# gsgen3d/gsgen

Measured on AMD Instinct MI355X. Metric: fwd+bwd renders/sec (800x800, 100k Gaussians), higher is better.
Workload: dtype f32

## Files before the change

gsgen_amd/_capi.py:

```python
import ctypes as C
import os

_HERE = os.path.dirname(os.path.abspath(__file__))
DEFAULT_LIB = os.environ.get("GSGEN_HIP_LIB") or os.path.join(_HERE, "lib", "libgsgen_hip.so")

u32, f32, vp, i32, sz = C.c_uint32, C.c_float, C.c_void_p, C.c_int, C.c_size_t



class ShView(C.Structure):
    _fields_ = [("mean", vp), ("cov", vp), ("start", vp), ("end", vp), ("gaussian_ids", vp),
                ("tile_order", vp), ("topleft", vp), ("c2w", vp), ("bg_rgb", vp),
                ("pixel_size_x", f32), ("pixel_size_y", f32), ("out", vp), ("T", vp),
                ("segment_workspace", vp), ("grad_out", vp), ("grad_mean", vp), ("grad_cov", vp), ("route_report", vp),
                ("no_fallback", u32), ("pixel_size_dev", vp)]


class RgbdView(C.Structure):
    _fields_ = [("mean", vp), ("cov", vp), ("depth", vp), ("start", vp), ("end", vp), ("gaussian_ids", vp),
                ("tile_order", vp), ("topleft", vp), ("pixel_size_x", f32), ("pixel_size_y", f32), ("out6", vp),
                ("T", vp), ("grad_out6", vp), ("grad_mean", vp), ("grad_cov", vp), ("grad_chan6", vp),
                ("grad_rgb", vp), ("grad_depth", vp), ("grad_opacity", vp), ("grad_depth2", vp),
                ("out_rgb", vp), ("out_depth", vp), ("out_opacity", vp), ("out_depth2", vp), ("bg_rgb", vp), ("grad_bg", vp),
                ("depth_variance", u32), ("chol", vp), ("pixel_size_dev", vp)]


class GeometryView(C.Structure):
    _fields_ = [("cam", vp), ("mean2d", vp), ("cov2d", vp), ("depth", vp), ("mask", vp), ("gaussian_ids", vp),
                ("start", vp), ("end", vp), ("total", vp), ("workspace", vp), ("workspace_bytes", sz), ("D_cap", u32),
                ("zero_grad_mean2d", vp), ("zero_grad_cov2d", vp), ("zero_grad_chan6", vp), ("pair_report", vp), ("chol", vp),
# ... 113 lines not shown
    "gsgen_image_loss_backward": [vp, vp, u32, u32, u32, u32, u32, f32, i32, vp, vp, vp, sz, vp],
    "gsgen_marching_cubes": [vp, u32, u32, u32, f32, vp, u32, vp, u32, vp, vp, sz, vp],
    "gsgen_depth_loss_forward": [vp, vp, sz, vp, sz, u32, u32, vp, vp, sz, vp],
    "gsgen_depth_loss_backward": [vp, vp, sz, vp, sz, u32, u32, vp, vp, vp, vp, sz, vp],
}
OPTIONAL_SIZE_FUNCS = {
    "gsgen_knn_workspace_bytes": [u32, u32],
    "gsgen_knn_query_workspace_bytes": [u32, u32, u32],
    "gsgen_density_grid_workspace_bytes": [u32, u32],
    "gsgen_fps_workspace_bytes": [u32, u32, u32, u32, i32],
    "gsgen_image_loss_workspace_bytes": [u32, u32, u32, u32, u32, i32],
    "gsgen_marching_cubes_workspace_bytes": [u32, u32, u32],
    "gsgen_depth_loss_workspace_bytes": [u32, u32],
}
EXPORTS = sorted(list(SIGNATURES) + list(SIZE_FUNCS) + list(PTR_FUNCS) + list(OPTIONAL_SIGNATURES) + list(OPTIONAL_SIZE_FUNCS)
                 + ["gsgen_version", "gsgen_error_string", "gsgen_kernel_variant", "gsgen_sh_poly_applies", "gsgen_emit_stage_capacity"])


class GsgenError(RuntimeError):
    pass


class Lib:
    def __init__(self, path=None):
        path = path or DEFAULT_LIB
        if not os.path.exists(path):
            raise ImportError(
                f"{path} not found: build the HIP extension first (python -m gsgen_amd.build). "
                "gsgen_amd has no CPU fallback.")
        self.path = path
        if path == DEFAULT_LIB or "libgsgen_hip" in os.path.basename(path):
# ... 35 lines not shown
        def call(*args):
            rc = fn(*args)
            if rc != 0:
                raise GsgenError(f"{name} failed: {err(rc).decode()} (code {rc})")
        call.__name__ = name
        return call

    def version(self):
        return self.cdll.gsgen_version().decode()

    def emit_stage_capacity(self):
        fn = self.cdll.gsgen_emit_stage_capacity
        fn.restype, fn.argtypes = u32, []
        return int(fn())

    def sh_poly_applies(self, sh_l1_bound, max_pixel_size, bands=4):
        fn = self.cdll.gsgen_sh_poly_applies
        fn.argtypes, fn.restype = [f32, f32, u32], i32
        return bool(fn(float(sh_l1_bound), float(max_pixel_size), int(bands)))

    def kernel_variant(self, stage, bands=4, n_segments=1):
        fn = self.cdll.gsgen_kernel_variant
        fn.argtypes, fn.restype = [C.c_char_p, u32, u32, C.c_char_p, sz], i32
        buf = C.create_string_buffer(192)
        n = fn(stage.encode(), bands, n_segments, buf, len(buf))
        if n <= 0:
            raise ValueError(f"unknown compositing stage {stage!r}")
        return buf.value.decode()


# ... 11 lines not shown
```

gsgen_amd/batch.py:

```python
import ctypes

import numpy as np
import torch

from . import _capi
from . import renderer as R
from .renderer import _p, PairListOverflow


ACTIVATION_CODES = {"nothing": 0, "exp": 1, "sigmoid": 2, "abs": 3, "relu": 4, "softplus": 5, "biased_relu": 6, "biased_abs": 7}
TORCH_ACTIVATIONS = {"nothing": lambda x: x, "exp": torch.exp, "sigmoid": torch.sigmoid, "abs": torch.abs, "relu": torch.relu,
                     "softplus": torch.nn.functional.softplus, "biased_relu": lambda x: torch.relu(x) + 1e-3,
                     "biased_abs": lambda x: torch.abs(x) + 1e-3}

_EXT = [False]


def _batch_ext():
    if _EXT[0] is False:
        import glob
        import importlib.util
        import os
        hits = glob.glob(os.path.join(os.path.dirname(os.path.abspath(__file__)), "ext", "_gsbatch.*.so"))
        mod = None
# ... 47 lines not shown
        out_p, T_p = out.data_ptr(), T.data_ptr()
        kind = "sh" if C > 0 else "rgb"
        gsh = torch.empty(br._Np + (col.numel() + 3) // 4 * 4, device=dev, dtype=torch.float32)
        with _on(dev):
            parts = br._fork(B)
            views = br._geometry(kind, B, parts, mean, qvec, svec, gsh, stats)
            bg_p = _p(bg_rgb)
            cis = br._cis
            if C > 0:
                rr, nf = br._route_args
                for i in range(B):
                    ci, v = cis[i], views[i]
                    v.pixel_size_x, v.pixel_size_y = 1.0 / ci.fx, 1.0 / ci.fy
                    v.T, v.bg_rgb, v.out = T_p + 4 * H * W * i, bg_p, out_p + 12 * H * W * i
                    v.route_report, v.no_fallback = rr, nf
            else:
                for i in range(B):
                    ci, v = cis[i], views[i]
                    v.pixel_size_x, v.pixel_size_y = 1.0 / ci.fx, 1.0 / ci.fy
                    v.T, v.out6 = T_p + 4 * H * W * i, out_p + 12 * H * W * i
            nth, ntw = br.slots[0].nth, br.slots[0].ntw
            for k, (lo, n, s) in enumerate(parts):
                if C > 0:
                    lib.vol_render_sh_batch_routed(n, _sub(views, lo, n), N, _p(col), _p(alpha), 16, nth, ntw, H, W, C,
                                                   thresh, br.segments, _p(br._sh_bound), _p(br._sh_rows), _p(br._bws[k]), s)
                else:
                    lib.vol_render_rgb_batch(n, _sub(views, lo, n), N, _p(col), _p(alpha), 16, nth, ntw, H, W, thresh,
                                             _p(br._bws[k]), s)
            br._join(parts)
        if C == 0 and bg_rgb is not None:
# ... 162 lines not shown
class BatchRenderer:

    def __init__(self, N, W, H, device, max_batch, D_cap=None, segments=1, strict=False, pipeline=False, device_cameras=False):
        self.N, self.W, self.H, self.device = N, W, H, torch.device(device)
        self.device_cameras = bool(device_cameras)
        self.segments = int(segments)
        self.strict = bool(strict)
        if pipeline not in ("auto", True, False):
            raise ValueError("pipeline: 'auto', True or False")
        self.pipeline = pipeline
        self._totals = torch.zeros(max_batch, device=device, dtype=torch.int32)
        self._report = R.PairCountReport(max_batch)
        self._route = R.PairCountReport(1)
        self._route_clean = 0
        self._route_args = (None, 0)
        self.strict = self.strict or self._report.unmapped
        self._gen = np.zeros(1, np.int64)
        self._plans = {}
        self.use_ext = True
        self._sh_bound = self._sh_rows = None
        self._table_cache = {}
        self._depths = torch.empty(max_batch, N, device=device, dtype=torch.float32)
        self.slots = [R.FrameBuffers(N, W, H, device, D_cap=D_cap, segments=self.segments, total=self._totals[i:i + 1],
                                     depth=self._depths[i].view(N, 1), report=(self._report, i), strict=self.strict)
                      for i in range(max_batch)]
        self._ptr_tabs = {}
        self._side = None
        self._ev = None
        lib = _capi.load()
        self._Np = (N + 3) // 4 * 4
# ... 305 lines not shown
        self._sh_bound = self._sh_rows = None
        if int(C) == 4 and sh_basis == "auto":
            if sh_l1_bound is not None:
                if not (isinstance(sh_l1_bound, torch.Tensor) and sh_l1_bound.is_cuda and sh_l1_bound.dtype == torch.float32
                        and sh_l1_bound.numel() == 1):
                    raise ValueError("sh_l1_bound: a 1-float CUDA tensor (the bound lives on the device; "
                                     "renderer.sh_l1_bound_device computes it)")
                if verify_bound:
                    R.verify_sh_l1_bound(col, sh_l1_bound)
                self._sh_bound = sh_l1_bound
            else:
                self._sh_rows = self._measure_bound(col)
                self._sh_bound = self._smax if self._sh_rows is self._rows else None
        self._begin_batch(B)
        self._route_args = self._route_mode() if (int(C) == 4 and self._sh_rows is not None) else (None, 0)
        fast = self._plan("sh" if int(C) > 0 else "rgb", B)
        if fast is not None:
            self._last_parts = [(0, B)]
            va = fast[1]
            va["pixel_size_x"][:B] = 1.0 / self._intr[:B, 0]
            va["pixel_size_y"][:B] = 1.0 / self._intr[:B, 1]
            if int(C) > 0:
                va["route_report"][:B] = self._route_args[0] or 0
                va["no_fallback"][:B] = self._route_args[1]
            out, T = _batch_ext().render(fast[0], mean, qvec, svec, alpha, col, bg_rgb, int(C), float(thresh), bool(detach_depth),
                                         self._sh_bound, self._sh_rows, *self._stats_args(stats))
            return out, T
        return _render_batch.apply(mean, qvec, svec, alpha, col, cams, self, B, int(C), bg_rgb, float(thresh),
                                   bool(detach_depth), stats)

    def _route_mode(self):
        rep = self._route
        if rep.ptr(0) is None:
            return None, 0
        seen = int(rep._np[0, 0])
        rep._np[0, 0] = 0
        self._route_clean = 0 if seen else self._route_clean + 1
        return rep.ptr(0), 1 if (self._route_clean >= 3 and not self.device_cameras) else 0

# ... 54 lines not shown
```

gsgen_amd/csrc/composite.hip:

```cpp
#include "composite_common.hpp"
#include <stdio.h>
#include <string.h>
#include <string>
#include <type_traits>
#include <vector>

namespace gs {

template <int MODE, int CB, int KB = kBatch, bool WITH_COL = true>
struct Stage {
  using TR = Traits<MODE, CB>;
  float mx[KB], my[KB], a[KB];
  float c0[KB], c1[KB], c2[KB], c3[KB];
  float p0[KB], p1[KB], p2[KB];
  int id[KB];
  alignas(16) float col[WITH_COL ? KB * TR::NCOLP : 4];
};

template <int MODE, int CB, int NT, int KB = kBatch, bool SCALE = false, bool WITH_COL = true>
__device__ __forceinline__ void stage_batch(Stage<MODE, CB, KB, WITH_COL> &S, const CompParams &p, int list_base,
                                            int nb) {
  using TR = Traits<MODE, CB>;
  const int t = (int)threadIdx.x;
  static_assert(KB <= NT, "one thread per staged record");
// ... 419 lines not shown
  }
}
template <int NT>
__device__ __forceinline__ uint32_t exact_tier_mask(const CompParams &p, const int *ids, int nb, int t, uint32_t *slot) {
  bool bad = false;
  if (p.sh_rows != nullptr && t < nb) bad = !poly_row_ok(p.sh_rows[ids[t]], fmaxf(fabsf(p.psx), fabsf(p.psy)));
  const uint32_t m = (uint32_t)__ballot((int)bad);
  if constexpr (NT == 64) {
    (void)slot;
    return m;
  } else {
    if (t == 0) *slot = m;
    return 0u;
  }
}
template <int CB, bool POLY>
struct FwdShVecShared {
  static constexpr int KB = POLY ? 32 : kBatch;
  Stage<MODE_SH, CB, KB, !POLY> S;
  alignas(16) float Vs[POLY ? kPolyNB * 16 : 4];
  alignas(16) float Ws[POLY ? KB * 3 * kPolyStride : 4];
  uint32_t exact_mask;
  float tay_ok[POLY ? KB * 3 : 1];
};
template <int CB, int PPL, int NB, bool PERSIST = false, bool TRACK = true>
__device__ __forceinline__ void composite_fwd_sh_vec_tile(const CompParams &p, uint32_t bid, FwdShVecShared<CB, (NB > 0)> &sm) {
  static_assert(PPL == 4 || PPL == 2, "pixel pairs: 2 or 4 pixels per lane");
  constexpr bool POLY = NB > 0;
  static_assert(!POLY || (NB == kPolyNB && CB == 4), "polynomial basis: SH degree 3");
  constexpr int MODE = MODE_SH;
  using TR = Traits<MODE, CB>;
  constexpr int NT = 256 / PPL, ROWS = NT / 16, NP = PPL / 2;
  constexpr int CCP = POLY ? NB : TR::CCP, NPAIR = CCP / 2;
  constexpr int KB = FwdShVecShared<CB, POLY>::KB;
  auto &S = sm.S;
  float *const Vs = sm.Vs;
  float *const Ws = sm.Ws;
  int tx, ty;
  if (!block_tile(p, tx, ty, bid)) return;
  const int tile = ty * p.ntw + tx;
  const int st = p.start[tile];
  const int n = (st < 0) ? 0 : (p.end[tile] - st);
  const int t = tile_thread_index<PERSIST>();
  const int lx = t & 15, ly0 = t >> 4;
  const int gx = tx * kTile + lx;

  bool valid[PPL];
  int gy[PPL], stop[PPL];
#pragma unroll
  for (int j = 0; j < PPL; ++j) {
    gy[j] = ty * kTile + ly0 + j * ROWS;
    valid[j] = (gx < p.W) && (gy[j] < p.H);
    stop[j] = valid[j] ? n : 0;
  }
  if constexpr (POLY) {
    if (t == 0 && p.tile_flags != nullptr) p.tile_flags[tile] = 0;
  }
  const bool has_bg = p.bg != nullptr;
  float bgv[3] = {0.0f, 0.0f, 0.0f};
  if (has_bg) { bgv[0] = p.bg[0]; bgv[1] = p.bg[1]; bgv[2] = p.bg[2]; }
  if (st == kListOverflow) {
#pragma unroll
    for (int j = 0; j < PPL; ++j)
      if (valid[j]) poison_pixel<3>(p, (size_t)gy[j] * p.W + gx);
    return;
  }
  if (n == 0) {
    if (p.bg != nullptr || p.fill_empty) {
#pragma unroll
      for (int j = 0; j < PPL; ++j)
        if (valid[j]) {
// ... 12 lines not shown
  }

  const float px = pixel_coord(p.topleft[0], gx, p.psx);
  v2f py2[NP];
#pragma unroll
  for (int j = 0; j < PPL; ++j) py2[j >> 1][j & 1] = pixel_coord(p.topleft[1], gy[j], p.psy);
  v2f Yp[POLY ? 1 : PPL][POLY ? 1 : NPAIR];
  const float pu = poly_offset(lx);
  const v2f pu2 = splat2(pu);
  v2f pv2[NP];
#pragma unroll
  for (int jp = 0; jp < NP; ++jp) pv2[jp] = v2f{poly_offset(ly0 + (2 * jp) * ROWS), poly_offset(ly0 + (2 * jp + 1) * ROWS)};
  if constexpr (POLY) {
    static_assert(KB * 3 * kPolyNB >= kPolyNodes * 16, "node scratch fits the coefficient buffer");
    poly_tile_setup<NT>(p, tx, ty, Ws, Vs);
  } else {
    float R[9];
#pragma unroll
    for (int i = 0; i < 9; ++i) R[i] = p.rot[i];
#pragma unroll
    for (int j = 0; j < PPL; ++j) {
      const float pyj = py2[j >> 1][j & 1];
      float Yf[CCP];
      sh_basis_of_pixel<CB>(R, px, pyj, Yf);
#pragma unroll
      for (int k = 0; k < NPAIR; ++k) Yp[j][k] = v2f{Yf[2 * k], Yf[2 * k + 1]};
      __builtin_amdgcn_sched_barrier(0);
    }
  }

  v2f acc2[NP][3], Tr2[NP];
#pragma unroll
  for (int jp = 0; jp < NP; ++jp) {
#pragma unroll
    for (int c = 0; c < 3; ++c) acc2[jp][c] = v2f{0.0f, 0.0f};
    Tr2[jp] = v2f{valid[2 * jp] ? 1.0f : -1.0f, valid[2 * jp + 1] ? 1.0f : -1.0f};
  }
  auto alive = [&](int j) { return !(Tr2[j >> 1][j & 1] < p.thresh); };
  const bool seg_out = p.nseg > 1 && p.ckpt != nullptr;
  const bool track_stop = TRACK && p.stop != nullptr;

  uint32_t exact_mask = 0u;
  uint32_t tay_mask = 0u;
  for (int base = 0; base < n; base += KB) {
    const int nb = min(KB, n - base);
    if (base > 0) __syncthreads();
    stage_batch<MODE, CB, NT, KB, true, !POLY>(S, p, st + base, nb);
    if constexpr (POLY) {
      if (p.sh_rows != nullptr) {
        exact_mask = exact_tier_mask<NT>(p, S.id, nb, t, &sm.exact_mask);
        __syncthreads();
        if constexpr (NT != 64) exact_mask = sm.exact_mask;
        exact_mask = (uint32_t)__builtin_amdgcn_readfirstlane((int)exact_mask);
        if (__popcll((unsigned long long)exact_mask) * kExactTierShare > nb) {
          if (t == 0 && p.route_report != nullptr) report_crowded_tile(p.route_report);
          if (!p.no_fallback) {
            if (t == 0 && p.tile_flags != nullptr) p.tile_flags[tile] = 1;
            return;
          }
        }
      } else {
        exact_mask = 0u;
        __syncthreads();
      }
      poly_transform<NT, KB>(p.col, S.id, Vs, Ws, nb, sm.tay_ok);
      __syncthreads();
      tay_mask = (uint32_t)__builtin_amdgcn_readfirstlane((int)(taylor_mask(sm.tay_ok, nb) & ~exact_mask));
      taylor_convert<NT>(Ws, tay_mask, nb);
      __syncthreads();
    } else {
      __syncthreads();
    }

    for (int g = 0; g < nb; ++g) {
      bool any_alive = false;
#pragma unroll
      for (int j = 0; j < PPL; ++j) any_alive |= alive(j);
      if (!wave_any(any_alive)) break;
      const int e_idx = base + g;
      if (seg_out && (e_idx % kSegLen) == 0 && e_idx > 0 && e_idx / kSegLen < p.nseg) {
#pragma unroll
        for (int j = 0; j < PPL; ++j)
          p.ckpt[((size_t)tile * p.nseg + e_idx / kSegLen) * 256 + (ly0 + j * ROWS) * 16 + lx] =
              make_float4(Tr2[j >> 1][j & 1], acc2[j >> 1][0][j & 1], acc2[j >> 1][1][j & 1], acc2[j >> 1][2][j & 1]);
// ... 102 lines not shown
          const bool was[2] = {alive(2 * jp), alive(2 * jp + 1)};
          Tr2[jp] = Tr2[jp] * one_minus2(ag2[jp]);
#pragma unroll
          for (int e = 0; e < 2; ++e)
            if (was[e] && !alive(2 * jp + e)) stop[2 * jp + e] = base + g + 1;
        }
      } else {
#pragma unroll
        for (int jp = 0; jp < NP; ++jp) Tr2[jp] = Tr2[jp] * one_minus2(ag2[jp]);
      }
    }
    bool any_alive = false;
#pragma unroll
    for (int j = 0; j < PPL; ++j) any_alive |= alive(j);
    if (__syncthreads_or((int)any_alive) == 0) break;
  }

#pragma unroll
  for (int j = 0; j < PPL; ++j) {
    if (!valid[j]) continue;
    const size_t pix = (size_t)gy[j] * p.W + gx;
    const float Tj = Tr2[j >> 1][j & 1];
    float *o = p.out + 3 * pix;
#pragma unroll
    for (int c = 0; c < 3; ++c) {
      const float a = acc2[j >> 1][c][j & 1];
      o[c] = has_bg ? a + bgv[c] * Tj : a;
    }
    if (p.T != nullptr) p.T[pix] = Tj;
  }
// ... 98 lines not shown
      const CompParams *pp = &plist[view];
      const PixelSizes<PSD> ps = view_pixel_sizes<PSD>(*pp);
      if (per_tile ? !tile_flagged(*pp, b - base) : poly_route(pp->sh_bound, ps.x(), ps.y())) continue;
      const CompParams p = view_params<PSD>(*pp, ps);
      composite_fwd_sh_vec_tile<4, PPL, 0, true>(p, b - base, sm);
      __syncthreads();
    }
  } else if constexpr (NB == kPolyNB && BATCH) {
    __shared__ FwdShVecShared<4, true> sm;
    const CompParams *pp = &plist[batch_view(p_arg, bid)];
    const PixelSizes<PSD> ps = view_pixel_sizes<PSD>(*pp);
    const bool view_ok = pp->sh_bound != nullptr && poly_route(pp->sh_bound, ps.x(), ps.y());
    if (pp->sh_rows == nullptr && !view_ok) return;
    CompParams p = view_params<PSD>(*pp, ps);
    if (view_ok) p.sh_rows = nullptr;
    composite_fwd_sh_vec_tile<4, PPL, kPolyNB, false, TRACK>(p, bid, sm);
  } else {
    const CompParams *pp = BATCH ? &plist[batch_view(p_arg, bid)] : &p_arg;
    const CompParams p = view_params<PSD>(*pp, view_pixel_sizes<PSD>(*pp));
    __shared__ FwdShVecShared<CB, (NB > 0)> sm;
    composite_fwd_sh_vec_tile<CB, PPL, NB>(p, bid, sm);
  }
}

template <int MODE, int CB, int PPL, int TS>
__global__ void __launch_bounds__(TS * TS / PPL)
k_composite_bwd_pixel(CompParams p) {
  const uint32_t bid = blockIdx.x, grid = gridDim.x;
  using TR = Traits<MODE, CB>;
  constexpr int NT = TS * TS / PPL;
  static_assert(NT >= kBatch && NT % 64 == 0, "a staging round needs one thread per record");
// ... 210 lines not shown
    if (__syncthreads_or((int)any_alive) == 0) break;
  }
}


template <int CB, int PPL, bool POLY>
struct BwdShVecShared {
  static constexpr int KB = 32;
  static constexpr int NT = 256 / PPL, NP = PPL / 2;
  Stage<MODE_SH, CB, KB, !POLY> S;
  v2f go_s[!POLY ? 3 * NP * NT : 1];
  alignas(16) float Vs[POLY ? kPolyNB * 16 : 4];
  alignas(16) float Ws[POLY ? KB * 3 * kPolyStride : 4];
  float gw_s[POLY ? 3 * 8 : 1];
  float tay_ok[POLY ? KB * 3 : 1];
};
template <int CB, int PPL, int NB, bool PERSIST = false, bool MOM = false>
__device__ __forceinline__ void composite_bwd_sh_vec_tile(const CompParams &p, uint32_t bid, uint32_t grid,
                                                          BwdShVecShared<CB, PPL, (NB > 0)> &sm) {
  static_assert(PPL == 4 || PPL == 2, "pixel pairs: 2 or 4 pixels per lane");
  constexpr bool POLY = NB > 0;
  static_assert(!POLY || (NB == kPolyNB && CB == 4 && PPL == 4), "polynomial basis: SH degree 3, one wavefront per tile");
  constexpr int MODE = MODE_SH;
  using TR = Traits<MODE, CB>;
  constexpr int NT = 256 / PPL, ROWS = NT / 16, NP = PPL / 2;
  constexpr int CCP = POLY ? NB : TR::CCP, NPAIR = CCP / 2, NSH = 3 * CCP;
  static_assert(NSH % 2 == 0, "component layout");
  constexpr int KB = BwdShVecShared<CB, PPL, POLY>::KB;
  auto &S = sm.S;
  v2f *const go_s = sm.go_s;
  float *const Vs = sm.Vs;
  float *const Ws = sm.Ws;
  float *const gw_s = sm.gw_s;
  const int nseg = p.nseg > 1 ? p.nseg : 1;
  const uint32_t tiles_grid = grid / (uint32_t)nseg;
  const int seg = (int)(bid / tiles_grid);
// ... 35 lines not shown
  if constexpr (TR::CCP != TR::CC) {
    for (int e = t; e < KB * TR::NCOLP; e += NT) S.col[e] = 0.0f;
    __syncthreads();
  }

  v2f Yp[POLY ? 1 : PPL][POLY ? 1 : NPAIR];
  float *geo_base = nullptr;
  uint32_t geo_stride = 0u;
  const float pu = poly_offset(lx);
  const v2f pu2 = splat2(pu);
  v2f pv2[NP];
#pragma unroll
  for (int jp = 0; jp < NP; ++jp) pv2[jp] = v2f{poly_offset(ly0 + (2 * jp) * ROWS), poly_offset(ly0 + (2 * jp + 1) * ROWS)};
  if constexpr (POLY) {
    static_assert(!POLY || KB * 3 * kPolyNB >= kPolyNodes * 16, "node scratch fits the coefficient buffer");
    poly_tile_setup<NT>(p, tx, ty, Ws, Vs);
    {
      const int comp = sep16_comp(lane), cls = comp >> 3, slot = comp & 7;
      if (sep16_owner(lane)) {
        if (cls < 3 && slot == 6) {
          geo_base = cls == 0 ? p.g_mean : p.g_cov + (cls == 1 ? 0 : (MOM ? 2 : 3));
          geo_stride = cls == 0 ? 2u : 4u;
        } else if (cls == 3) {
          geo_base = slot == 0 ? p.g_mean + 1 : (slot == 1 ? p.g_cov + 1 : p.g_alpha);
          geo_stride = slot == 0 ? 2u : (slot == 1 ? 4u : 1u);
        }
      } else if (!MOM && cls == 3 && slot == 1) {
        geo_base = p.g_cov + 2;
        geo_stride = 4u;
      }
    }
// ... 32 lines not shown
    R2[jp] = fma2(go2[jp][2], rem2[jp][2], fma2(go2[jp][1], rem2[jp][1], go2[jp][0] * rem2[jp][0]));
    pvsq2[jp] = pv2[jp] * pv2[jp];
  }
  if constexpr (!POLY) {
#pragma unroll
    for (int jp = 0; jp < NP; ++jp)
#pragma unroll
      for (int c = 0; c < 3; ++c) go_s[(c * NP + jp) * NT + t] = go2[jp][c];
  }
  auto alive = [&](int j) { return !(Tr2[j >> 1][j & 1] < p.thresh); };

  uint32_t exact_mask = 0u, tay_mask = 0u;
  for (int base = e_lo; base < e_hi; base += KB) {
    const int nb = min(KB, e_hi - base);
    if (base > e_lo) __syncthreads();
    stage_batch<MODE, CB, NT, KB, true, !POLY>(S, p, st + base, nb);
    __syncthreads();
    if constexpr (POLY) {
      exact_mask = (uint32_t)__builtin_amdgcn_readfirstlane((int)exact_tier_mask<NT>(p, S.id, nb, t, nullptr));
      poly_transform<NT, KB>(p.col, S.id, Vs, Ws, nb, sm.tay_ok);
      __syncthreads();
      tay_mask = (uint32_t)__builtin_amdgcn_readfirstlane((int)(taylor_mask(sm.tay_ok, nb) & ~exact_mask));
      taylor_convert<NT>(Ws, tay_mask, nb);
      __syncthreads();
    }

    for (int g = 0; g < nb; ++g) {
      bool any_alive = false;
#pragma unroll
      for (int j = 0; j < PPL; ++j) any_alive |= alive(j);
      if (!wave_any(any_alive)) break;

      auto uni = [&](float v) { return !POLY ? wave_uniform(v) : v; };
      const float r_mx = uni(S.mx[g]), r_my = uni(S.my[g]), r_a = uni(S.a[g]), r_c0 = uni(S.c0[g]), r_c1 = uni(S.c1[g]),
                  r_c2 = uni(S.c2[g]), r_c3 = uni(S.c3[g]), r_p0 = uni(S.p0[g]), r_p1 = uni(S.p1[g]);
      const float x = px - r_mx;
      v2f y2[NP], G2[NP], ag2[NP], tx2[NP], ty2[NP];
      bool any_con = false;
      float guard_dist = 0.0f;
// ... 270 lines not shown
      const CompParams *pp = &plist[view];
      const PixelSizes<PSD> ps = view_pixel_sizes<PSD>(*pp);
      if (per_tile ? !tile_flagged(*pp, (b - base) % tiles_grid) : poly_route(pp->sh_bound, ps.x(), ps.y())) continue;
      const CompParams p = view_params<PSD>(*pp, ps);
      composite_bwd_sh_vec_tile<4, 4, 0, true, MOM>(p, b - base, per, sm);
      __syncthreads();
    }
  } else if constexpr (NB == kPolyNB && BATCH) {
    __shared__ BwdShVecShared<4, 4, true> sm;
    const CompParams *pp = &plist[batch_view(p_arg, bid, &grid)];
    const PixelSizes<PSD> ps = view_pixel_sizes<PSD>(*pp);
    const bool view_ok = pp->sh_bound != nullptr && poly_route(pp->sh_bound, ps.x(), ps.y());
    if (pp->sh_rows == nullptr && !view_ok) return;
    CompParams p = view_params<PSD>(*pp, ps);
    if (view_ok) p.sh_rows = nullptr;
    composite_bwd_sh_vec_tile<4, 4, kPolyNB, false, MOM>(p, bid, grid, sm);
  } else {
    const CompParams *pp = BATCH ? &plist[batch_view(p_arg, bid, &grid)] : &p_arg;
    const CompParams p = view_params<PSD>(*pp, view_pixel_sizes<PSD>(*pp));
    __shared__ BwdShVecShared<CB, PPL, (NB > 0)> sm;
    composite_bwd_sh_vec_tile<CB, PPL, NB, false, MOM>(p, bid, grid, sm);
  }
}

template <int MODE, bool BATCH = false>
__global__ void __launch_bounds__(64) GS_WAVES_PER_EU(6)
k_composite_fwd_chan_vec(CompParams p_arg, ViewPack<BATCH> pack) {
  const CompParams *plist = pack.table();
  static_assert(MODE == MODE_RGB || MODE == MODE_SCALAR || MODE == MODE_RGBD, "post-activation channel modes");
  uint32_t bid = blockIdx.x;
  const CompParams p = BATCH ? view_params(plist[batch_view(p_arg, bid)]) : p_arg;
// ... 750 lines not shown
    p.stop = reinterpret_cast<int *>(p.ckpt + (size_t)n_tiles_h * n_tiles_w * 256 * n_segments);
  }
  hipStream_t s = (hipStream_t)stream;
  switch (C) {
    case 1: return launch_fwd<MODE_SH, 1>(p, s);
    case 2: return launch_fwd<MODE_SH, 2>(p, s);
    case 3: return launch_fwd<MODE_SH, 3>(p, s);
    default: return launch_fwd<MODE_SH, 4>(p, s);
  }
}

static int fill_view_params(uint32_t n_views, const gsgen_sh_view *views, const float *sh_coeffs,
                            const float *alpha, float *g_sh, float *g_alpha, uint32_t ntw, uint32_t nth,
                            uint32_t H, uint32_t W, float thresh, uint32_t n_segments, bool backward,
                            const float *sh_bound, std::vector<CompParams> &ps, const float *sh_rows = nullptr,
                            uint8_t *tile_flags = nullptr) {
  ps.assign(n_views, CompParams{});
  for (uint32_t b = 0; b < n_views; ++b) {
    const gsgen_sh_view &v = views[b];
    if (!v.start || !v.end || !v.out || !v.c2w) return GSGEN_EINVAL;
    if ((v.tile_order == nullptr) != (views[0].tile_order == nullptr)) return GSGEN_EINVAL;
    if (n_segments > 1 && v.segment_workspace == nullptr) return GSGEN_EINVAL;
    if (backward && (!v.grad_out || !v.grad_mean || !v.grad_cov)) return GSGEN_EINVAL;
    if ((v.pixel_size_dev == nullptr) != (views[0].pixel_size_dev == nullptr)) return GSGEN_EINVAL;
    CompParams &p = ps[b];
    p.mean = v.mean; p.cov = v.cov; p.col = sh_coeffs; p.alpha = alpha;
    p.start = v.start; p.end = v.end; p.ids = v.gaussian_ids; p.topleft = v.topleft; p.rot = v.c2w;
    p.ntw = (int)ntw; p.nth = (int)nth; p.H = (int)H; p.W = (int)W;
    p.psx = v.pixel_size_x; p.psy = v.pixel_size_y; p.thresh = thresh;
    p.ps_dev = v.pixel_size_dev;
    p.tile_order = v.tile_order;
    p.n_hi = 0x7fffffff;
    p.sh_bound = sh_bound;
    p.sh_rows = sh_rows;
    p.tile_flags = (sh_rows != nullptr && tile_flags != nullptr) ? tile_flags + (size_t)b * ntw * nth : nullptr;
    p.route_report = sh_rows != nullptr ? v.route_report : nullptr;
    p.no_fallback = (sh_rows != nullptr && views[0].no_fallback) ? 1 : 0;
    if (backward) {
      p.final_img = v.out; p.grad_out = v.grad_out;
      p.g_mean = v.grad_mean; p.g_cov = v.grad_cov; p.g_col = g_sh; p.g_alpha = g_alpha;
    } else {
      p.bg = v.bg_rgb; p.out = v.out; p.T = v.T;
      p.fill_empty = 1;
    }
    if (n_segments > 1) {
      p.nseg = (int)n_segments;
      p.ckpt = reinterpret_cast<float4 *>(v.segment_workspace);
      p.stop = reinterpret_cast<int *>(p.ckpt + (size_t)nth * ntw * 256 * n_segments);
    }
  }
  return 0;
}
// ... 163 lines not shown
  return sh_l1_pass<true>(N, sh_coeffs, C, nullptr, bound, n_violations, (hipStream_t)stream);
}

int gsgen_sh_poly_applies(float sh_l1_bound, float max_pixel_size, uint32_t C) {
  return (C == 4 && poly_ok(sh_l1_bound, max_pixel_size)) ? 1 : 0;
}

static bool batch_can_be_polynomial(const std::vector<CompParams> &ps) {
  if (!ps.empty() && ps[0].ps_dev != nullptr) return true;
  for (const CompParams &p : ps)
    if (poly_ok(1.0f / 16.0f, fmaxf(fabsf(p.psx), fabsf(p.psy)))) return true;
  return false;
}

size_t gsgen_sh_batch_workspace_bytes(uint32_t n_views) { return 2 * (size_t)n_views * sizeof(CompParams); }
size_t gsgen_sh_batch_workspace_bytes_routed(uint32_t n_views, uint32_t n_tiles) {
  return gsgen_sh_batch_workspace_bytes(n_views) + (((size_t)n_views * n_tiles + 15u) & ~(size_t)15u);
}

int gsgen_vol_render_sh_batch(uint32_t n_views, const gsgen_sh_view *views, uint32_t N,
                              const float *sh_coeffs, const float *alpha, uint32_t tile_size,
                              uint32_t n_tiles_h, uint32_t n_tiles_w, uint32_t H, uint32_t W, uint32_t C,
                              float thresh, uint32_t n_segments, void *batch_workspace,
                              gsgen_stream_t stream) {
  return gsgen_vol_render_sh_batch_bounded(n_views, views, N, sh_coeffs, alpha, tile_size, n_tiles_h, n_tiles_w, H, W, C,
                                           thresh, n_segments, nullptr, batch_workspace, stream);
}

int gsgen_vol_render_sh_batch_bounded(uint32_t n_views, const gsgen_sh_view *views, uint32_t N,
                                      const float *sh_coeffs, const float *alpha, uint32_t tile_size,
                                      uint32_t n_tiles_h, uint32_t n_tiles_w, uint32_t H, uint32_t W, uint32_t C,
                                      float thresh, uint32_t n_segments, const float *sh_l1_bound, void *batch_workspace,
// ... 3 lines not shown
}

int gsgen_vol_render_sh_batch_routed(uint32_t n_views, const gsgen_sh_view *views, uint32_t N,
                                     const float *sh_coeffs, const float *alpha, uint32_t tile_size,
                                     uint32_t n_tiles_h, uint32_t n_tiles_w, uint32_t H, uint32_t W, uint32_t C,
                                     float thresh, uint32_t n_segments, const float *sh_l1_bound, const float *sh_row_bounds,
                                     void *batch_workspace, gsgen_stream_t stream) {
  if (tile_size != 16) return GSGEN_EUNSUPPORTED;
  if (C < 1 || C > 4) return GSGEN_EUNSUPPORTED;
  if (n_views == 0) return 0;
  if (!views || !batch_workspace) return GSGEN_EINVAL;
  if (n_views > 65535) return GSGEN_EINVAL;
  (void)N;
  std::vector<CompParams> ps;
  uint8_t *flags = reinterpret_cast<uint8_t *>(batch_workspace) + gsgen_sh_batch_workspace_bytes(n_views);
  if (int e = fill_view_params(n_views, views, sh_coeffs, alpha, nullptr, nullptr, n_tiles_w, n_tiles_h, H, W,
                               thresh, n_segments, false, C == 4 ? sh_l1_bound : nullptr, ps, C == 4 ? sh_row_bounds : nullptr, flags))
    return e;
  const bool bounded = C == 4 && (sh_l1_bound != nullptr || sh_row_bounds != nullptr) && batch_can_be_polynomial(ps);
  if (!bounded)
    for (CompParams &p : ps) { p.sh_bound = nullptr; p.sh_rows = nullptr; p.tile_flags = nullptr; }
  hipStream_t s = (hipStream_t)stream;
  return launch_fwd_sh_batch((int)C, ps.data(), n_views, s, bounded);
}

int gsgen_vol_render_backward_sh_batch(uint32_t n_views, const gsgen_sh_view *views, uint32_t N,
                                       const float *sh_coeffs, const float *alpha, float *grad_sh_coeffs,
                                       float *grad_alpha, uint32_t tile_size, uint32_t n_tiles_h,
                                       uint32_t n_tiles_w, uint32_t H, uint32_t W, uint32_t C, float thresh,
                                       uint32_t n_segments, void *batch_workspace, gsgen_stream_t stream) {
  return gsgen_vol_render_backward_sh_batch_bounded(n_views, views, N, sh_coeffs, alpha, grad_sh_coeffs, grad_alpha, tile_size,
                                                    n_tiles_h, n_tiles_w, H, W, C, thresh, n_segments, nullptr, batch_workspace,
                                                    stream);
}

int gsgen_vol_render_backward_sh_batch_bounded(uint32_t n_views, const gsgen_sh_view *views, uint32_t N,
// ... 8 lines not shown
}

static int backward_sh_batch_routed(bool moments, uint32_t n_views, const gsgen_sh_view *views, uint32_t N,
                                    const float *sh_coeffs, const float *alpha, float *grad_sh_coeffs,
                                    float *grad_alpha, uint32_t tile_size, uint32_t n_tiles_h,
                                    uint32_t n_tiles_w, uint32_t H, uint32_t W, uint32_t C, float thresh,
                                    uint32_t n_segments, const float *sh_l1_bound, const float *sh_row_bounds,
                                    void *batch_workspace, gsgen_stream_t stream) {
  if (tile_size != 16) return GSGEN_EUNSUPPORTED;
  if (C < 1 || C > 4) return GSGEN_EUNSUPPORTED;
  if (n_views == 0 || N == 0) return 0;
  if (!views || !batch_workspace || !grad_sh_coeffs || !grad_alpha) return GSGEN_EINVAL;
  if (n_views > 65535) return GSGEN_EINVAL;
  std::vector<CompParams> ps;
  uint8_t *flags = reinterpret_cast<uint8_t *>(batch_workspace) + gsgen_sh_batch_workspace_bytes(n_views);
  if (int e = fill_view_params(n_views, views, sh_coeffs, alpha, grad_sh_coeffs, grad_alpha, n_tiles_w,
                               n_tiles_h, H, W, thresh, n_segments, true, C == 4 ? sh_l1_bound : nullptr, ps,
                               C == 4 ? sh_row_bounds : nullptr, flags))
    return e;
  const bool bounded = C == 4 && (sh_l1_bound != nullptr || sh_row_bounds != nullptr) && batch_can_be_polynomial(ps);
  if (!bounded)
    for (CompParams &p : ps) { p.sh_bound = nullptr; p.sh_rows = nullptr; p.tile_flags = nullptr; }
  hipStream_t s = (hipStream_t)stream;
  return launch_bwd_sh_batch((int)C, ps.data(), n_views, s, bounded, moments);
}
int gsgen_vol_render_backward_sh_batch_routed(uint32_t n_views, const gsgen_sh_view *views, uint32_t N,
                                              const float *sh_coeffs, const float *alpha, float *grad_sh_coeffs,
                                              float *grad_alpha, uint32_t tile_size, uint32_t n_tiles_h,
                                              uint32_t n_tiles_w, uint32_t H, uint32_t W, uint32_t C, float thresh,
                                              uint32_t n_segments, const float *sh_l1_bound, const float *sh_row_bounds,
                                              void *batch_workspace, gsgen_stream_t stream) {
  return backward_sh_batch_routed(false, n_views, views, N, sh_coeffs, alpha, grad_sh_coeffs, grad_alpha, tile_size, n_tiles_h,
                                  n_tiles_w, H, W, C, thresh, n_segments, sh_l1_bound, sh_row_bounds, batch_workspace, stream);
}
int gsgen_vol_render_backward_sh_batch_routed_moments(uint32_t n_views, const gsgen_sh_view *views, uint32_t N,
                                                      const float *sh_coeffs, const float *alpha, float *grad_sh_coeffs,
                                                      float *grad_alpha, uint32_t tile_size, uint32_t n_tiles_h,
// ... 142 lines not shown
```

gsgen_amd/csrc/composite_common.hpp:

```cpp
#pragma once
#include "common.hpp"
#include "../../include/gsgen_hip.h"

namespace gs {

enum : int { MODE_RGB = 0, MODE_SCALAR = 1, MODE_SH = 2, MODE_RGBD = 3 };
constexpr int kBatch = 64;

struct CompParams {
  const float *mean, *cov, *col, *alpha;
  const float *depth;
  const int *start, *end, *ids;
  const float *topleft, *rot, *bg;
  float *out, *T;
  const float *final_img, *grad_out;
  float *g_mean, *g_cov, *g_col, *g_alpha;
  int ntw, nth, H, W;
  float psx, psy, thresh;
  const uint32_t *tile_order;
  int n_lo, n_hi;
  float4 *ckpt;
  int *stop;
  int nseg;
  int tile_side;
  const float *go_rgb, *go_d, *go_o, *go_z2;
  const float *sh_bound;
  const float *sh_rows;
  uint8_t *tile_flags;
  uint32_t vgrid;
  int fill_empty;
  float *pl_rgb, *pl_d, *pl_o, *pl_z;
  float *g_bg;
  int zvar;
  const float *chol;
  uint32_t *route_report;
  int no_fallback;
  const float *ps_dev;
};
__device__ __forceinline__ CompParams view_params(const CompParams &src) {
  CompParams p = src;
  if (p.ps_dev != nullptr) {
    p.psx = p.ps_dev[0];
    p.psy = p.ps_dev[1];
  }
  return p;
}
constexpr int kSegLen = 32;

__device__ __forceinline__ bool block_tile(const CompParams &p, int &tx, int &ty, uint32_t bid) {
  if (p.tile_order != nullptr) {
    const uint32_t t = p.tile_order[bid];
    tx = (int)(t % (uint32_t)p.ntw);
// ... 373 lines not shown
```

include/gsgen_hip.h:

```cpp
#ifndef GSGEN_HIP_H
#define GSGEN_HIP_H
#include <stddef.h>
#include <stdint.h>

#ifdef __cplusplus
extern "C" {
#endif
#if defined(__GNUC__)
#pragma GCC visibility push(default)
#endif

typedef void *gsgen_stream_t;

#define GSGEN_EUNSUPPORTED (-2)
#define GSGEN_EINVAL (-3)
#define GSGEN_EWORKSPACE (-4)

const char *gsgen_version(void);
const char *gsgen_error_string(int code);
int gsgen_kernel_variant(const char *stage, uint32_t C, uint32_t n_segments, char *out, size_t out_bytes);

int gsgen_culling_gaussian_bsphere(uint32_t N, const float *mean, const float *qvec,
                                   const float *svec, const float *normal ,
                                   const float *pts , uint8_t *mask, float thresh,
// ... 222 lines not shown

typedef struct gsgen_sh_view {
  const float *mean, *cov;
  const int *start, *end, *gaussian_ids;
  const uint32_t *tile_order;
  const float *topleft, *c2w;
  const float *bg_rgb;
  float pixel_size_x, pixel_size_y;
  float *out, *T;
  void *segment_workspace;
  const float *grad_out;
  float *grad_mean, *grad_cov;
  uint32_t *route_report;
  uint32_t no_fallback;
  const float *pixel_size_dev;
} gsgen_sh_view;
size_t gsgen_sh_batch_workspace_bytes(uint32_t n_views);
int gsgen_vol_render_sh_batch(uint32_t n_views, const gsgen_sh_view *views, uint32_t N,
                              const float *sh_coeffs, const float *alpha, uint32_t tile_size,
                              uint32_t n_tiles_h, uint32_t n_tiles_w, uint32_t H, uint32_t W, uint32_t C,
                              float thresh, uint32_t n_segments, void *batch_workspace,
                              gsgen_stream_t stream);
int gsgen_vol_render_backward_sh_batch(uint32_t n_views, const gsgen_sh_view *views, uint32_t N,
                                       const float *sh_coeffs, const float *alpha, float *grad_sh_coeffs,
                                       float *grad_alpha, uint32_t tile_size, uint32_t n_tiles_h,
                                       uint32_t n_tiles_w, uint32_t H, uint32_t W, uint32_t C, float thresh,
                                       uint32_t n_segments, void *batch_workspace, gsgen_stream_t stream);

int gsgen_sh_l1_bound(uint32_t N, const float *sh_coeffs, uint32_t C, float *out ,
                      gsgen_stream_t stream);
// ... 24 lines not shown
                                         const int *end, const int *gaussian_ids, const float *out,
                                         float *grad_mean, float *grad_cov, float *grad_sh_coeffs,
                                         float *grad_alpha, const float *grad_out, const float *topleft,
                                         const float *c2w, uint32_t tile_size, uint32_t n_tiles_h,
                                         uint32_t n_tiles_w, float pixel_size_x, float pixel_size_y,
                                         uint32_t H, uint32_t W, uint32_t C, float thresh,
                                         const float *bg_rgb, const uint32_t *tile_order,
                                         const void *segment_workspace, uint32_t n_segments,
                                         const float *sh_l1_bound , gsgen_stream_t stream);

int gsgen_sh_l1_bound_rows(uint32_t N, const float *sh_coeffs, uint32_t C, float *out_max ,
                           float *out_rows , gsgen_stream_t stream);
int gsgen_sh_l1_bound_rows_running(uint32_t N, const float *sh_coeffs, uint32_t C, float *running_max ,
                                   float *out_rows , gsgen_stream_t stream);
size_t gsgen_sh_batch_workspace_bytes_routed(uint32_t n_views, uint32_t n_tiles);
int gsgen_vol_render_sh_batch_routed(uint32_t n_views, const gsgen_sh_view *views, uint32_t N,
                                     const float *sh_coeffs, const float *alpha, uint32_t tile_size,
                                     uint32_t n_tiles_h, uint32_t n_tiles_w, uint32_t H, uint32_t W, uint32_t C,
                                     float thresh, uint32_t n_segments, const float *sh_l1_bound ,
                                     const float *sh_row_bounds , void *batch_workspace,
                                     gsgen_stream_t stream);
int gsgen_vol_render_backward_sh_batch_routed(uint32_t n_views, const gsgen_sh_view *views, uint32_t N,
                                              const float *sh_coeffs, const float *alpha, float *grad_sh_coeffs,
                                              float *grad_alpha, uint32_t tile_size, uint32_t n_tiles_h,
                                              uint32_t n_tiles_w, uint32_t H, uint32_t W, uint32_t C, float thresh,
                                              uint32_t n_segments, const float *sh_l1_bound, const float *sh_row_bounds,
                                              void *batch_workspace, gsgen_stream_t stream);
int gsgen_vol_render_backward_sh_batch_routed_moments(uint32_t n_views, const gsgen_sh_view *views, uint32_t N,
                                                      const float *sh_coeffs, const float *alpha, float *grad_sh_coeffs,
                                                      float *grad_alpha, uint32_t tile_size, uint32_t n_tiles_h,
// ... 127 lines not shown
```

Before: 7438.

## Save forward per-tile staged SH batches for backward reuse in routed polynomial path

The forward polynomial SH compositing kernel now writes each tile's poly setup and its first five staged Gaussian batches (records, ids, converted coefficients, masks) to a workspace region. The backward kernel checks a per-tile header (output pointer, start, count) and reloads these blocks instead of restaging and recomputing them. This is meant to cut redundant staging and Taylor conversion work in the backward pass. In exchange the forward pass does extra global writes and the workspace grows. Reuse is turned off when no gradients are needed or when there are multiple segments.

```diff
diff --git a/gsgen_amd/_capi.py b/gsgen_amd/_capi.py
--- a/gsgen_amd/_capi.py
+++ b/gsgen_amd/_capi.py
@@ -13,7 +13,7 @@
                 ("tile_order", vp), ("topleft", vp), ("c2w", vp), ("bg_rgb", vp),
                 ("pixel_size_x", f32), ("pixel_size_y", f32), ("out", vp), ("T", vp),
                 ("segment_workspace", vp), ("grad_out", vp), ("grad_mean", vp), ("grad_cov", vp), ("route_report", vp),
-                ("no_fallback", u32), ("pixel_size_dev", vp)]
+                ("no_fallback", u32), ("pixel_size_dev", vp), ("no_batch_reuse", u32)]
 
 
 class RgbdView(C.Structure):
@@ -157,7 +157,8 @@
     "gsgen_depth_loss_workspace_bytes": [u32, u32],
 }
 EXPORTS = sorted(list(SIGNATURES) + list(SIZE_FUNCS) + list(PTR_FUNCS) + list(OPTIONAL_SIGNATURES) + list(OPTIONAL_SIZE_FUNCS)
-                 + ["gsgen_version", "gsgen_error_string", "gsgen_kernel_variant", "gsgen_sh_poly_applies", "gsgen_emit_stage_capacity"])
+                 + ["gsgen_version", "gsgen_error_string", "gsgen_kernel_variant", "gsgen_sh_poly_applies", "gsgen_emit_stage_capacity",
+                    "gsgen_sh_batch_saved_batches"])
 
 
 class GsgenError(RuntimeError):
@@ -223,6 +224,11 @@
         fn.restype, fn.argtypes = u32, []
         return int(fn())
 
+    def sh_batch_saved_batches(self):
+        fn = self.cdll.gsgen_sh_batch_saved_batches
+        fn.restype, fn.argtypes = u32, []
+        return int(fn())
+
     def sh_poly_applies(self, sh_l1_bound, max_pixel_size, bands=4):
         fn = self.cdll.gsgen_sh_poly_applies
         fn.argtypes, fn.restype = [f32, f32, u32], i32
diff --git a/gsgen_amd/batch.py b/gsgen_amd/batch.py
--- a/gsgen_amd/batch.py
+++ b/gsgen_amd/batch.py
@@ -85,6 +85,7 @@
                     v.pixel_size_x, v.pixel_size_y = 1.0 / ci.fx, 1.0 / ci.fy
                     v.T, v.bg_rgb, v.out = T_p + 4 * H * W * i, bg_p, out_p + 12 * H * W * i
                     v.route_report, v.no_fallback = rr, nf
+                    v.no_batch_reuse = br._no_reuse
             else:
                 for i in range(B):
                     ci, v = cis[i], views[i]
@@ -277,6 +278,7 @@
         self._route = R.PairCountReport(1)
         self._route_clean = 0
         self._route_args = (None, 0)
+        self._no_reuse = 0
         self.strict = self.strict or self._report.unmapped
         self._gen = np.zeros(1, np.int64)
         self._plans = {}
@@ -612,6 +614,7 @@
                 self._sh_bound = self._smax if self._sh_rows is self._rows else None
         self._begin_batch(B)
         self._route_args = self._route_mode() if (int(C) == 4 and self._sh_rows is not None) else (None, 0)
+        self._no_reuse = 0 if (torch.is_grad_enabled() and any(x.requires_grad for x in (mean, qvec, svec, alpha, col))) else 1
         fast = self._plan("sh" if int(C) > 0 else "rgb", B)
         if fast is not None:
             self._last_parts = [(0, B)]
@@ -621,6 +624,7 @@
             if int(C) > 0:
                 va["route_report"][:B] = self._route_args[0] or 0
                 va["no_fallback"][:B] = self._route_args[1]
+                va["no_batch_reuse"][:B] = self._no_reuse
             out, T = _batch_ext().render(fast[0], mean, qvec, svec, alpha, col, bg_rgb, int(C), float(thresh), bool(detach_depth),
                                          self._sh_bound, self._sh_rows, *self._stats_args(stats))
             return out, T
diff --git a/gsgen_amd/csrc/composite.hip b/gsgen_amd/csrc/composite.hip
--- a/gsgen_amd/csrc/composite.hip
+++ b/gsgen_amd/csrc/composite.hip
@@ -457,6 +457,66 @@
     return 0u;
   }
 }
+constexpr int kSaveBatches = 5;
+constexpr int kSaveKB = 32;
+constexpr int kSaveRecQuads = 9 * kSaveKB / 4;
+constexpr int kSaveIdQuads = kSaveKB / 4;
+constexpr int kSaveRowQuads = kSaveKB * 3 * kPolyStride / 4;
+constexpr int kSaveBlockQuads = kSaveRecQuads + kSaveIdQuads + kSaveRowQuads + 1;
+constexpr int kSaveHeadQuads = 2 + kPolyNB * 16 / 4;
+constexpr int kSaveTileQuads = kSaveHeadQuads + kSaveBatches * kSaveBlockQuads;
+static_assert(kSaveRecQuads == 72 && kSaveRecQuads + kSaveIdQuads + kSaveRowQuads == 4 * 64 + 16, "a block: four passes of a wavefront and a quarter");
+__device__ __forceinline__ float4 *save_tile(const CompParams &p, int tile) { return p.save + (size_t)tile * kSaveTileQuads; }
+__device__ __forceinline__ float4 *save_block(const CompParams &p, int tile, int blk) {
+  return save_tile(p, tile) + kSaveHeadQuads + blk * kSaveBlockQuads;
+}
+template <class StageT>
+__device__ __forceinline__ float4 *save_lds_quad(StageT &S, float *Ws, int q) {
+  static_assert(sizeof(S.mx) == kSaveKB * 4 && offsetof(StageT, p1) == 8 * sizeof(S.mx) && offsetof(StageT, id) % 16 == 0,
+                "nine contiguous record arrays of 32 floats, 16-byte aligned ids");
+  float *f = q < kSaveRecQuads ? S.mx + 4 * q
+                               : (q < kSaveRecQuads + kSaveIdQuads ? reinterpret_cast<float *>(S.id) + 4 * (q - kSaveRecQuads)
+                                                                   : Ws + 4 * (q - kSaveRecQuads - kSaveIdQuads));
+  return reinterpret_cast<float4 *>(f);
+}
+__device__ __forceinline__ void save_write_header(const CompParams &p, int tile, int st, int n) {
+  uint32_t *h = reinterpret_cast<uint32_t *>(save_tile(p, tile));
+  const uint64_t a = (uint64_t)reinterpret_cast<uintptr_t>(p.out);
+  h[0] = (uint32_t)a; h[1] = (uint32_t)(a >> 32); h[2] = (uint32_t)st; h[3] = (uint32_t)n; h[4] = 0u;
+}
+template <class StageT>
+__device__ __forceinline__ void save_store_block(float4 *blk, StageT &S, float *Ws, int t, uint32_t exact_mask, uint32_t tay_mask) {
+#pragma unroll
+  for (int k = 0; k < 4; ++k) blk[64 * k + t] = *save_lds_quad(S, Ws, 64 * k + t);
+  if (t < 16) blk[256 + t] = *save_lds_quad(S, Ws, 256 + t);
+  if (t == 16) {
+    uint32_t *m = reinterpret_cast<uint32_t *>(blk + kSaveBlockQuads - 1);
+    m[0] = exact_mask; m[1] = tay_mask;
+  }
+}
+__device__ __forceinline__ int save_match(const CompParams &p, int tile, int st, int n) {
+  if (p.save == nullptr) return 0;
+  const uint32_t *h = reinterpret_cast<const uint32_t *>(save_tile(p, tile));
+  const uint64_t a = (uint64_t)reinterpret_cast<uintptr_t>(p.final_img);
+  const bool same = h[0] == (uint32_t)a && h[1] == (uint32_t)(a >> 32) && h[2] == (uint32_t)st && h[3] == (uint32_t)n;
+  const uint32_t k = h[4];
+  return __builtin_amdgcn_readfirstlane(same ? (int)(k < (uint32_t)kSaveBatches ? k : (uint32_t)kSaveBatches) : 0);
+}
+template <class StageT>
+__device__ __forceinline__ void save_load_block(const float4 *blk, StageT &S, float *Ws, int t, uint32_t &exact_mask, uint32_t &tay_mask) {
+  float4 q[5];
+#pragma unroll
+  for (int k = 0; k < 4; ++k) q[k] = blk[64 * k + t];
+  q[4] = blk[256 + (t & 15)];
+  const uint32_t *m = reinterpret_cast<const uint32_t *>(blk + kSaveBlockQuads - 1);
+  const uint32_t em = m[0], tm = m[1];
+#pragma unroll
+  for (int k = 0; k < 4; ++k) *save_lds_quad(S, Ws, 64 * k + t) = q[k];
+  if (t < 16) *save_lds_quad(S, Ws, 256 + t) = q[4];
+  exact_mask = (uint32_t)__builtin_amdgcn_readfirstlane((int)em);
+  tay_mask = (uint32_t)__builtin_amdgcn_readfirstlane((int)tm);
+}
+
 template <int CB, bool POLY>
 struct FwdShVecShared {
   static constexpr int KB = POLY ? 32 : kBatch;
@@ -466,10 +526,11 @@
   uint32_t exact_mask;
   float tay_ok[POLY ? KB * 3 : 1];
 };
-template <int CB, int PPL, int NB, bool PERSIST = false, bool TRACK = true>
+template <int CB, int PPL, int NB, bool PERSIST = false, bool TRACK = true, bool SAVE = false>
 __device__ __forceinline__ void composite_fwd_sh_vec_tile(const CompParams &p, uint32_t bid, FwdShVecShared<CB, (NB > 0)> &sm) {
   static_assert(PPL == 4 || PPL == 2, "pixel pairs: 2 or 4 pixels per lane");
   constexpr bool POLY = NB > 0;
+  static_assert(!SAVE || (POLY && PPL == 4 && !PERSIST), "saved batches: the polynomial form, one wavefront per tile");
   static_assert(!POLY || (NB == kPolyNB && CB == 4), "polynomial basis: SH degree 3");
   constexpr int MODE = MODE_SH;
   using TR = Traits<MODE, CB>;
@@ -498,6 +559,9 @@
   }
   if constexpr (POLY) {
     if (t == 0 && p.tile_flags != nullptr) p.tile_flags[tile] = 0;
+    if constexpr (SAVE) {
+      if (t == 0 && p.save != nullptr) save_write_header(p, tile, st, n);
+    }
   }
   const bool has_bg = p.bg != nullptr;
   float bgv[3] = {0.0f, 0.0f, 0.0f};
@@ -540,6 +604,9 @@
   if constexpr (POLY) {
     static_assert(KB * 3 * kPolyNB >= kPolyNodes * 16, "node scratch fits the coefficient buffer");
     poly_tile_setup<NT>(p, tx, ty, Ws, Vs);
+    if constexpr (SAVE) {
+      if (p.save_blocks > 0 && t < kPolyNB * 16 / 4) save_tile(p, tile)[2 + t] = reinterpret_cast<const float4 *>(Vs)[t];
+    }
   } else {
     float R[9];
 #pragma unroll
@@ -568,7 +635,8 @@
 
   uint32_t exact_mask = 0u;
   uint32_t tay_mask = 0u;
-  for (int base = 0; base < n; base += KB) {
+  int base = 0;
+  for (; base < n; base += KB) {
     const int nb = min(KB, n - base);
     if (base > 0) __syncthreads();
     stage_batch<MODE, CB, NT, KB, true, !POLY>(S, p, st + base, nb);
@@ -594,6 +662,10 @@
       tay_mask = (uint32_t)__builtin_amdgcn_readfirstlane((int)(taylor_mask(sm.tay_ok, nb) & ~exact_mask));
       taylor_convert<NT>(Ws, tay_mask, nb);
       __syncthreads();
+      if constexpr (SAVE) {
+        static_assert(!SAVE || (KB == kSaveKB && NT == 64), "a block is a batch of one wavefront");
+        if (base < p.save_blocks * KB) save_store_block(save_block(p, tile, base / KB), S, Ws, t, exact_mask, tay_mask);
+      }
     } else {
       __syncthreads();
     }
@@ -726,6 +798,10 @@
 #pragma unroll
     for (int j = 0; j < PPL; ++j) any_alive |= alive(j);
     if (__syncthreads_or((int)any_alive) == 0) break;
+  }
+  if constexpr (SAVE) {
+    if (t == 0 && p.save_blocks > 0)
+      reinterpret_cast<uint32_t *>(save_tile(p, tile))[4] = (uint32_t)min(min(base / KB + 1, (n + KB - 1) / KB), p.save_blocks);
   }
 
 #pragma unroll
@@ -854,7 +930,7 @@
     if (pp->sh_rows == nullptr && !view_ok) return;
     CompParams p = view_params<PSD>(*pp, ps);
     if (view_ok) p.sh_rows = nullptr;
-    composite_fwd_sh_vec_tile<4, PPL, kPolyNB, false, TRACK>(p, bid, sm);
+    composite_fwd_sh_vec_tile<4, PPL, kPolyNB, false, TRACK, PPL == 4>(p, bid, sm);
   } else {
     const CompParams *pp = BATCH ? &plist[batch_view(p_arg, bid)] : &p_arg;
     const CompParams p = view_params<PSD>(*pp, view_pixel_sizes<PSD>(*pp));
@@ -1095,12 +1171,14 @@
   alignas(16) float Ws[POLY ? KB * 3 * kPolyStride : 4];
   float gw_s[POLY ? 3 * 8 : 1];
   float tay_ok[POLY ? KB * 3 : 1];
+  int n_saved;
 };
-template <int CB, int PPL, int NB, bool PERSIST = false, bool MOM = false>
+template <int CB, int PPL, int NB, bool PERSIST = false, bool MOM = false, bool SAVE = false>
 __device__ __forceinline__ void composite_bwd_sh_vec_tile(const CompParams &p, uint32_t bid, uint32_t grid,
                                                           BwdShVecShared<CB, PPL, (NB > 0)> &sm) {
   static_assert(PPL == 4 || PPL == 2, "pixel pairs: 2 or 4 pixels per lane");
   constexpr bool POLY = NB > 0;
+  static_assert(!SAVE || (POLY && !PERSIST), "saved batches: the polynomial form");
   static_assert(!POLY || (NB == kPolyNB && CB == 4 && PPL == 4), "polynomial basis: SH degree 3, one wavefront per tile");
   constexpr int MODE = MODE_SH;
   using TR = Traits<MODE, CB>;
@@ -1166,7 +1244,18 @@
   for (int jp = 0; jp < NP; ++jp) pv2[jp] = v2f{poly_offset(ly0 + (2 * jp) * ROWS), poly_offset(ly0 + (2 * jp + 1) * ROWS)};
   if constexpr (POLY) {
     static_assert(!POLY || KB * 3 * kPolyNB >= kPolyNodes * 16, "node scratch fits the coefficient buffer");
-    poly_tile_setup<NT>(p, tx, ty, Ws, Vs);
+    int n_saved = 0;
+    if constexpr (SAVE) {
+      static_assert(!SAVE || (KB == kSaveKB && NT == 64), "a block is a batch of one wavefront");
+      if (nseg == 1) n_saved = save_match(p, tile, st, n);
+      if (t == 0) sm.n_saved = n_saved;
+    }
+    if (n_saved > 0) {
+      if (t < kPolyNB * 16 / 4) reinterpret_cast<float4 *>(Vs)[t] = save_tile(p, tile)[2 + t];
+      __syncthreads();
+    } else {
+      poly_tile_setup<NT>(p, tx, ty, Ws, Vs);
+    }
     {
       const int comp = sep16_comp(lane), cls = comp >> 3, slot = comp & 7;
       if (sep16_owner(lane)) {
@@ -1229,6 +1318,12 @@
   for (int base = e_lo; base < e_hi; base += KB) {
     const int nb = min(KB, e_hi - base);
     if (base > e_lo) __syncthreads();
+    bool saved = false;
+    if constexpr (SAVE) saved = base < __builtin_amdgcn_readfirstlane(sm.n_saved) * KB;
+    if (saved) {
+      save_load_block(save_block(p, tile, base / KB), S, Ws, t, exact_mask, tay_mask);
+      __syncthreads();
+    } else {
     stage_batch<MODE, CB, NT, KB, true, !POLY>(S, p, st + base, nb);
     __syncthreads();
     if constexpr (POLY) {
@@ -1238,6 +1333,7 @@
       tay_mask = (uint32_t)__builtin_amdgcn_readfirstlane((int)(taylor_mask(sm.tay_ok, nb) & ~exact_mask));
       taylor_convert<NT>(Ws, tay_mask, nb);
       __syncthreads();
+    }
     }
 
     for (int g = 0; g < nb; ++g) {
@@ -1538,7 +1634,7 @@
     if (pp->sh_rows == nullptr && !view_ok) return;
     CompParams p = view_params<PSD>(*pp, ps);
     if (view_ok) p.sh_rows = nullptr;
-    composite_bwd_sh_vec_tile<4, 4, kPolyNB, false, MOM>(p, bid, grid, sm);
+    composite_bwd_sh_vec_tile<4, 4, kPolyNB, false, MOM, true>(p, bid, grid, sm);
   } else {
     const CompParams *pp = BATCH ? &plist[batch_view(p_arg, bid, &grid)] : &p_arg;
     const CompParams p = view_params<PSD>(*pp, view_pixel_sizes<PSD>(*pp));
@@ -2319,7 +2415,7 @@
                             const float *alpha, float *g_sh, float *g_alpha, uint32_t ntw, uint32_t nth,
                             uint32_t H, uint32_t W, float thresh, uint32_t n_segments, bool backward,
                             const float *sh_bound, std::vector<CompParams> &ps, const float *sh_rows = nullptr,
-                            uint8_t *tile_flags = nullptr) {
+                            uint8_t *tile_flags = nullptr, float4 *save = nullptr) {
   ps.assign(n_views, CompParams{});
   for (uint32_t b = 0; b < n_views; ++b) {
     const gsgen_sh_view &v = views[b];
@@ -2341,6 +2437,11 @@
     p.tile_flags = (sh_rows != nullptr && tile_flags != nullptr) ? tile_flags + (size_t)b * ntw * nth : nullptr;
     p.route_report = sh_rows != nullptr ? v.route_report : nullptr;
     p.no_fallback = (sh_rows != nullptr && views[0].no_fallback) ? 1 : 0;
+    if (p.tile_flags != nullptr && save != nullptr) {
+      const bool reuse = n_segments <= 1 && !v.no_batch_reuse;
+      p.save = (backward && !reuse) ? nullptr : save + (size_t)b * ntw * nth * kSaveTileQuads;
+      p.save_blocks = reuse ? kSaveBatches : 0;
+    }
     if (backward) {
       p.final_img = v.out; p.grad_out = v.grad_out;
       p.g_mean = v.grad_mean; p.g_cov = v.grad_cov; p.g_col = g_sh; p.g_alpha = g_alpha;
@@ -2534,8 +2635,16 @@
 }
 
 size_t gsgen_sh_batch_workspace_bytes(uint32_t n_views) { return 2 * (size_t)n_views * sizeof(CompParams); }
+static size_t sh_batch_flag_bytes(uint32_t n_views, uint32_t n_tiles) {
+  return gsgen_sh_batch_workspace_bytes(n_views) + (((size_t)n_views * n_tiles + 15u) & ~(size_t)15u);
+}
 size_t gsgen_sh_batch_workspace_bytes_routed(uint32_t n_views, uint32_t n_tiles) {
-  return gsgen_sh_batch_workspace_bytes(n_views) + (((size_t)n_views * n_tiles + 15u) & ~(size_t)15u);
+  return sh_batch_flag_bytes(n_views, n_tiles) + 16u + (size_t)n_views * n_tiles * kSaveTileQuads * sizeof(float4);
+}
+uint32_t gsgen_sh_batch_saved_batches(void) { return (uint32_t)kSaveBatches; }
+static float4 *sh_batch_save_region(void *batch_workspace, uint32_t n_views, uint32_t n_tiles) {
+  const uintptr_t a = reinterpret_cast<uintptr_t>(batch_workspace) + sh_batch_flag_bytes(n_views, n_tiles);
+  return reinterpret_cast<float4 *>((a + 15u) & ~(uintptr_t)15u);
 }
 
 int gsgen_vol_render_sh_batch(uint32_t n_views, const gsgen_sh_view *views, uint32_t N,
@@ -2569,12 +2678,13 @@
   (void)N;
   std::vector<CompParams> ps;
   uint8_t *flags = reinterpret_cast<uint8_t *>(batch_workspace) + gsgen_sh_batch_workspace_bytes(n_views);
+  float4 *save = (C == 4 && sh_row_bounds != nullptr) ? sh_batch_save_region(batch_workspace, n_views, n_tiles_h * n_tiles_w) : nullptr;
   if (int e = fill_view_params(n_views, views, sh_coeffs, alpha, nullptr, nullptr, n_tiles_w, n_tiles_h, H, W,
-                               thresh, n_segments, false, C == 4 ? sh_l1_bound : nullptr, ps, C == 4 ? sh_row_bounds : nullptr, flags))
+                               thresh, n_segments, false, C == 4 ? sh_l1_bound : nullptr, ps, C == 4 ? sh_row_bounds : nullptr, flags, save))
     return e;
   const bool bounded = C == 4 && (sh_l1_bound != nullptr || sh_row_bounds != nullptr) && batch_can_be_polynomial(ps);
   if (!bounded)
-    for (CompParams &p : ps) { p.sh_bound = nullptr; p.sh_rows = nullptr; p.tile_flags = nullptr; }
+    for (CompParams &p : ps) { p.sh_bound = nullptr; p.sh_rows = nullptr; p.tile_flags = nullptr; p.save = nullptr; p.save_blocks = 0; }
   hipStream_t s = (hipStream_t)stream;
   return launch_fwd_sh_batch((int)C, ps.data(), n_views, s, bounded);
 }
@@ -2613,13 +2723,14 @@
   if (n_views > 65535) return GSGEN_EINVAL;
   std::vector<CompParams> ps;
   uint8_t *flags = reinterpret_cast<uint8_t *>(batch_workspace) + gsgen_sh_batch_workspace_bytes(n_views);
+  float4 *save = (C == 4 && sh_row_bounds != nullptr) ? sh_batch_save_region(batch_workspace, n_views, n_tiles_h * n_tiles_w) : nullptr;
   if (int e = fill_view_params(n_views, views, sh_coeffs, alpha, grad_sh_coeffs, grad_alpha, n_tiles_w,
                                n_tiles_h, H, W, thresh, n_segments, true, C == 4 ? sh_l1_bound : nullptr, ps,
-                               C == 4 ? sh_row_bounds : nullptr, flags))
+                               C == 4 ? sh_row_bounds : nullptr, flags, save))
     return e;
   const bool bounded = C == 4 && (sh_l1_bound != nullptr || sh_row_bounds != nullptr) && batch_can_be_polynomial(ps);
   if (!bounded)
-    for (CompParams &p : ps) { p.sh_bound = nullptr; p.sh_rows = nullptr; p.tile_flags = nullptr; }
+    for (CompParams &p : ps) { p.sh_bound = nullptr; p.sh_rows = nullptr; p.tile_flags = nullptr; p.save = nullptr; p.save_blocks = 0; }
   hipStream_t s = (hipStream_t)stream;
   return launch_bwd_sh_batch((int)C, ps.data(), n_views, s, bounded, moments);
 }
diff --git a/gsgen_amd/csrc/composite_common.hpp b/gsgen_amd/csrc/composite_common.hpp
--- a/gsgen_amd/csrc/composite_common.hpp
+++ b/gsgen_amd/csrc/composite_common.hpp
@@ -36,6 +36,8 @@
   uint32_t *route_report;
   int no_fallback;
   const float *ps_dev;
+  float4 *save;
+  int save_blocks;
 };
 __device__ __forceinline__ CompParams view_params(const CompParams &src) {
   CompParams p = src;
diff --git a/include/gsgen_hip.h b/include/gsgen_hip.h
--- a/include/gsgen_hip.h
+++ b/include/gsgen_hip.h
@@ -260,6 +260,7 @@
   uint32_t *route_report;
   uint32_t no_fallback;
   const float *pixel_size_dev;
+  uint32_t no_batch_reuse;
 } gsgen_sh_view;
 size_t gsgen_sh_batch_workspace_bytes(uint32_t n_views);
 int gsgen_vol_render_sh_batch(uint32_t n_views, const gsgen_sh_view *views, uint32_t N,
@@ -314,6 +315,7 @@
 int gsgen_sh_l1_bound_rows_running(uint32_t N, const float *sh_coeffs, uint32_t C, float *running_max ,
                                    float *out_rows , gsgen_stream_t stream);
 size_t gsgen_sh_batch_workspace_bytes_routed(uint32_t n_views, uint32_t n_tiles);
+uint32_t gsgen_sh_batch_saved_batches(void);
 int gsgen_vol_render_sh_batch_routed(uint32_t n_views, const gsgen_sh_view *views, uint32_t N,
                                      const float *sh_coeffs, const float *alpha, uint32_t tile_size,
                                      uint32_t n_tiles_h, uint32_t n_tiles_w, uint32_t H, uint32_t W, uint32_t C,
```

New measurement: 7480, median of 6. No clear change (+0.6%).
